# Ladme/groan_rs

Hardware: AMD Instinct MI355X
Metric: frames/sec RMSD-fit, 1e6 atoms triclinic, 1/2/4/8 GPUs; HBM GB/s vs peak (higher is better)
Workload: dtype f32 (fp64 accumulators)

## Files before the change

### groan_rs_amd/csrc/gr_api.hip

```cpp
#include <hip/hip_runtime.h>

#include <cmath>
#include <cstdio>
#include <cstdlib>
#include <cstring>
#include <map>
#include <string>
#include <vector>

#include "../../include/groan_hip.h"
#include "gr_batch.h"
#include "gr_buf.h"
#include "gr_workers.h"
#include "gr_container.h"
#include "gr_kernels.h"
#include "gr_hot.h"
#include "gr_resident.h"
#include "gr_small.h"
#include "gr_xtc.h"
#include "gr_shape.h"
#include "gr_xtc_dev.h"
#include "gr_xtc_enc_dev.h"
#include "gr_trr.h"
#include "gr_cellgrid.h"
#include "gr_textio.h"
#include "gr_pool.h"
#include <set>
#include <thread>
#include <atomic>
#include <system_error>
#include <chrono>

#define GR_MAX_CHUNKS 256

namespace {

struct Group {
    std::vector<grc::Block> blocks;
    uint64_t n = 0;
    bool contiguous = true;
    uint32_t start = 0;
    uint32_t *idx_dev = nullptr;
    uint32_t *mask_dev = nullptr;
    bool walk_rw = false;
    bool masked = false;
    uint32_t span = 0;
};

}

struct GrWhole;

struct gr_ctx {
    int device = 0;
    hipStream_t stream = nullptr;
    hipStream_t copy_stream = nullptr;
    std::vector<hipEvent_t> ev_ready;
    std::vector<uint8_t> upload_pending;
    hipEvent_t ev_done_ring[64] = {};
    uint64_t done_gen = 0;
    std::vector<uint64_t> slot_gen;
    uint32_t *fuse_cnt = nullptr;
    int fuse = 1;
    uint64_t center_fallbacks = 0;
    uint32_t com_onepass_min = 4096;
    uint64_t n = 0, n_pad = 0;
    uint32_t n_slots = 0;
    size_t frame_stride = 0;
    float *frames = nullptr;
    float *aos_up = nullptr;
    float *aos_dl = nullptr;
    float *masses = nullptr;
    std::vector<float> masses_host;
    GrBox *boxes_dev = nullptr;
    GrBox *boxes_host = nullptr;
    std::vector<int> box_status;
    std::vector<uint8_t> box9_set;
    std::vector<float> box9_host;
    std::map<std::string, Group> groups;
    GrWhole *whole = nullptr;
    GrCenPartial *cen_partials = nullptr;
    GrAccPartial *acc_partials = nullptr;
    grbuf::Dev<double> fit_partials;
    int two_pass = 1;
    int masked_sel = 1;
    int rmsd_fast = 1;
    int rmsd_fast_sigmas = 6;
    uint32_t rmsd_fast_min = 16384;
    uint64_t rmsd_fast_frames = 0, rmsd_exact_redos = 0;
    int resident = 1;
    int pd_sym = 1;
    int res_wg_groups = 0;
    int res_streams = 0;
    int res_fill16 = 1;
    uint32_t res_last_streams = 0;
    int res_metro_ns = 1;
    int stream_wgs_cu = 0;
    int translate_rows = 1;
    int center_resident = 1;
    uint64_t cen_res_launches = 0, cen_res_redone = 0;
    int res_fit_last = 0;
    struct Metro { uint64_t shape = 0; double free_ns = 0, T_ns = 0, best_ns = 0, fail_ns = 0; uint32_t off_for = 0, held = 0; } metro;
    uint64_t res_metro_period_ns = 0, res_last_turn_ns = 0, res_late_permille = 0, res_sclk_mhz = 0;
    int wall_khz = 100000;
    uint32_t res_max_wgs = 0;
    int res_test_no_start = 0;
    uint32_t res_test_abort_at = 0xFFFFFFFFu;
    uint32_t res_skip = 0, res_backoff = 0;
    uint32_t *res_progress = nullptr;
    grbuf::Dev<unsigned long long> res_wgrec;
    unsigned long long *res_rec = nullptr;
    uint32_t *res_abort = nullptr;
    uint32_t *res_words_host = nullptr;
    struct ResOut { GrFrameState st[GR_MAX_BATCH]; uint32_t words[16]; alignas(64) uint32_t seq; };
    ResOut *res_out = nullptr, *res_out_dev = nullptr;
    uint32_t res_seq = 0;
    uint32_t res_checkin = 0, res_closed = 0;
    uint32_t res_late_seen[2] = { 0, 0 };
    uint64_t res_lean_segments = 0, res_sync_fallbacks = 0;
    GrShapeSet *shape_set_dev = nullptr;
    grbuf::Dev<unsigned long long> shape_mask_dev; grbuf::Pinned<unsigned long long> shape_mask_host;
    uint32_t res_epoch = 0;
    bool res_in_use = false;
    uint64_t res_launches = 0, res_handshake_misses = 0, res_aborts = 0, res_redone_frames = 0;
    GrFrameState *state_dev = nullptr;
    GrFrameState *state_host = nullptr;
    GrFrameState *small_state = nullptr, *small_state_dev = nullptr;
    uint32_t *small_flag = nullptr, *small_flag_dev = nullptr;
    uint32_t small_seq = 0;
    uint32_t small_max = GR_SMALL_MAX_DEFAULT;
    uint64_t small_calls = 0, small_sync_fallbacks = 0;
    uint32_t *bad_dev = nullptr;
    uint32_t *bad_host = nullptr;
    grbuf::Dev<float> pd_out;
    hipEvent_t ev0 = nullptr, ev1 = nullptr;
    hipEvent_t pev[6 * GR_MAX_BATCH] = {};
    uint32_t sub_batch = 256;
    uint32_t chunks = 0;
    uint32_t fit_wgs = 0;
    int profile = 0;
    double prof_ms[4] = { 0, 0, 0, 0 };
    uint64_t prof_launches[4] = { 0, 0, 0, 0 };
    uint64_t prof_frames[4] = { 0, 0, 0, 0 };
    uint32_t n_cus = 0;
    grbuf::Pinned<unsigned char> xtc_host[2]; grbuf::Dev<unsigned char> xtc_dev[2];
    hipEvent_t xtc_ev[2] = { nullptr, nullptr };
    hipEvent_t xtc_unpacked[2] = { nullptr, nullptr };
    hipStream_t unpack_stream = nullptr;
    uint32_t xtc_bank = 0;
    grbuf::Pinned<float> wr_host;
    grbuf::Dev<unsigned char> xe_dev[6];
    grbuf::Pinned<unsigned char> xe_host[2];
    int xtc_dev_encode = 1;
    uint64_t xtc_dev_frames = 0;
    int strict = 0;
    gr_rmsd_plan *in_flight = nullptr;
    uint32_t in_flight_s0 = 0, in_flight_n = 0;
    uint64_t epoch = 1;
    std::string err;
    uint64_t err_index = 0;
    uint64_t counts[2] = { 0, 0 };
};

struct Pending {
    bool active = false, any_ok = false, consistent = true, fused = false, resident = false, rmsd_fast = false;
    uint32_t res_metro_ns = 0; bool res_metro_auto = false;
    uint32_t s0 = 0, nb = 0, n_prof_groups = 0, res_stream = 0, res_streams = 1;
    int fit = 0;
    std::vector<int> pre;
    std::vector<uint64_t> pre_idx;
    std::vector<std::string> pre_msg;
    GrSel sel = {};
    uint64_t group_n = 0;
    bool has_group = false;
    bool small = false; uint32_t small_seq = 0;
    uint32_t res_seq = 0, res_epoch = 0; bool res_fresh = false;
#ifdef GR_EXP_TIMELINE
    unsigned long long *tl_dev = nullptr;
#endif
};

struct gr_rmsd_plan {
    gr_ctx *target = nullptr;
    Pending pend;
    std::string group;
    uint64_t n_ref = 0;
    float *p_dev = nullptr, *w_dev = nullptr;
    float *p_span_dev = nullptr;
    std::vector<grc::Block> ref_blocks;
    bool span_ok = false;
    std::vector<float> w_host;
    GrPlanDev dev = {};
    int exact = 0;
    bool fit_behind_small = false;
    uint32_t last_fallbacks = 0;
    bool resolved = false;
    uint64_t resolved_epoch = 0;
};

namespace {

thread_local std::string g_create_err;

#define HIPCHK(ctx, call)                                                                      \
    do {                                                                                       \
        hipError_t e_ = (call);                                                                \
        if (e_ != hipSuccess) {                                                                \
            (ctx)->err = std::string(#call) + ": " + hipGetErrorString(e_);                    \
            return GR_E_HIP;                                                                   \
        }                                                                                      \
    } while (0)

int fail(gr_ctx *c, int status, const std::string &msg, uint64_t index = 0) {
    c->err = msg; c->err_index = index; return status;
}

GrSel make_sel(const Group &g) {
    GrSel s;
    s.n = (uint32_t)g.n; s.contiguous = g.contiguous ? 1u : 0u; s.start = g.start; s.g0 = g.start >> 8; s.idx = g.idx_dev;
    s.masked = (g.masked && g.mask_dev) ? (g.walk_rw ? 3u : 1u) : 0u; s.span = g.contiguous ? (uint32_t)g.n : g.span; s.mask = g.mask_dev;
    return s;
}

uint32_t chunks_for(const GrSel &s) {
    const uint64_t units = s.contiguous ? ((uint64_t)s.n + 3) / 4 : (uint64_t)s.n;
    uint64_t c = units / ((uint64_t)GR_WG * 4);
    if (c < 1) c = 1;
    if (c > GR_MAX_CHUNKS) c = GR_MAX_CHUNKS;
    return (uint32_t)c;
}

uint32_t batch_chunks(const gr_ctx *c, const GrSel &s, uint32_t nf) {
    if (c->chunks) return c->chunks;
    const uint64_t units = ((uint64_t)(s.masked ? s.span : s.n) + 3) / 4;
    uint64_t by_work = units / GR_WG;
    if (by_work < 1) by_work = 1;
    uint64_t want = (1536 + nf - 1) / nf;
    if (want < 8) want = 8;
    uint64_t ch = want < by_work ? want : by_work;
    if (ch > GR_MAX_CHUNKS) ch = GR_MAX_CHUNKS;
    if (ch >= 8) ch &= ~(uint64_t)7;
    return (uint32_t)ch;
}

uint32_t fit_grid(const gr_ctx *c, uint32_t nf) {
    (void)nf;
    if (c->fit_wgs) return c->fit_wgs;
    const uint64_t tiles = (c->n + 255) >> 8;
    uint64_t gx = (tiles + GR_WG / 64 - 1) / (GR_WG / 64);
    if (gx >= 8) gx &= ~(uint64_t)7;
    return (uint32_t)(gx < 1 ? 1 : gx);
}

static const void *resident_fn(bool wmass, bool ubox, bool v, bool fl) {
#define GR_RES_FN(W, U, V, F) reinterpret_cast<const void *>(&k_fit_resident<W, U, V, F>)
    static const void *const fn[16] = {
        GR_RES_FN(false, false, false, false), GR_RES_FN(true, false, false, false), GR_RES_FN(false, true, false, false), GR_RES_FN(true, true, false, false),
        GR_RES_FN(false, false, true, false), GR_RES_FN(true, false, true, false), GR_RES_FN(false, true, true, false), GR_RES_FN(true, true, true, false),
        GR_RES_FN(false, false, false, true), GR_RES_FN(true, false, false, true), GR_RES_FN(false, true, false, true), GR_RES_FN(true, true, false, true),
        GR_RES_FN(false, false, true, true), GR_RES_FN(true, false, true, true), GR_RES_FN(false, true, true, true), GR_RES_FN(true, true, true, true) };
#undef GR_RES_FN
    return fn[(wmass ? 1 : 0) | (ubox ? 2 : 0) | (v ? 4 : 0) | (fl ? 8 : 0)];
}
static const void *resident_center_fn(bool ubox, bool fl) {
    static const void *const fn[4] = { reinterpret_cast<const void *>(&k_fit_resident<false, false, false, false, 1>), reinterpret_cast<const void *>(&k_fit_resident<false, true, false, false, 1>),
                                       reinterpret_cast<const void *>(&k_fit_resident<false, false, false, true, 1>), reinterpret_cast<const void *>(&k_fit_resident<false, true, false, true, 1>) };
    return fn[(ubox ? 1 : 0) | (fl ? 2 : 0)];
}
#ifndef GR_STREAM_WGS_CU_DEFAULT
#define GR_STREAM_WGS_CU_DEFAULT 8
// ... 147 lines not shown
    if (!ingest) return busy_check(c);
    if (c->in_flight && slot < c->in_flight_s0 + c->in_flight_n && c->in_flight_s0 < slot + n)
        return fail(c, GR_E_INVALID_ARG, "upload into a slot of the batch in flight: call gr_rmsd_batch_end first (or use the other half of the double buffer)");
    return GR_OK;
}

struct SlotUse {
    gr_ctx *c; uint32_t first, n;
    bool quiet = false;
    SlotUse(gr_ctx *ctx, uint32_t first_slot, uint32_t count = 1) : c(ctx), first(first_slot), n(count) {
        for (uint32_t s = first; s < first + n && s < c->n_slots; ++s)
            if (c->upload_pending[s]) { (void)hipStreamWaitEvent(c->stream, c->ev_ready[s], 0); c->upload_pending[s] = 0; }
    }
    ~SlotUse() {
        if (quiet) return;
        const uint64_t gen = ++c->done_gen;
        (void)hipEventRecord(c->ev_done_ring[gen % 64], c->stream);
        for (uint32_t s = first; s < first + n && s < c->n_slots; ++s) c->slot_gen[s] = gen;
    }
};

static hipError_t sync_ingest(gr_ctx *c) {
    hipError_t e = hipStreamSynchronize(c->copy_stream);
    if (e == hipSuccess && c->unpack_stream) e = hipStreamSynchronize(c->unpack_stream);
    return e;
}
static int slot_box_wait(gr_ctx *c, uint32_t slot) {
    if (c->ev_ready[slot]) HIPCHK(c, hipEventSynchronize(c->ev_ready[slot]));
    else HIPCHK(c, hipEventCreateWithFlags(&c->ev_ready[slot], hipEventDisableTiming));
    return GR_OK;
}
void box_fill(gr_ctx *c, uint32_t slot, const float *box9) {
    GrBox &b = c->boxes_host[slot];
    if (!box9) {
        gr_box_setup(nullptr, &b);
        c->box_status[slot] = GR_E_NO_BOX; c->box9_set[slot] = 0;
    } else {
        const int ok = gr_box_setup(box9, &b);
        memcpy(&c->box9_host[9 * (size_t)slot], box9, 9 * sizeof(float));
        c->box9_set[slot] = 1;
        if (!ok) c->box_status[slot] = GR_E_ZERO_BOX;
        else if (b.ncand > GR_MAX_CAND) c->box_status[slot] = GR_E_UNSUPPORTED_BOX;
        else c->box_status[slot] = GR_OK;
    }
}
int set_box(gr_ctx *c, uint32_t slot, const float *box9, hipStream_t on = nullptr) {
    box_fill(c, slot, box9);
    HIPCHK(c, hipMemcpyAsync(c->boxes_dev + slot, &c->boxes_host[slot], sizeof(GrBox), hipMemcpyHostToDevice, on ? on : c->stream));
    return GR_OK;
}

int set_boxes_same(gr_ctx *c, uint32_t first_slot, uint32_t n, const float *box9, hipStream_t on = nullptr) {
    if (n == 0) return GR_OK;
    float keep[9];
    if (box9) memcpy(keep, box9, sizeof keep);
    box_fill(c, first_slot, box9 ? keep : nullptr);
    for (uint32_t f = 1; f < n; ++f) {
        const uint32_t s = first_slot + f;
        c->boxes_host[s] = c->boxes_host[first_slot];
        c->box_status[s] = c->box_status[first_slot]; c->box9_set[s] = c->box9_set[first_slot];
        if (box9) memcpy(&c->box9_host[9 * (size_t)s], keep, sizeof keep);
    }
    HIPCHK(c, hipMemcpyAsync(c->boxes_dev + first_slot, c->boxes_host + first_slot, (size_t)n * sizeof(GrBox), hipMemcpyHostToDevice, on ? on : c->stream));
    return GR_OK;
}

int ensure_staging(gr_ctx *c, float **buf) {
    if (*buf) return GR_OK;
    HIPCHK(c, hipMalloc(buf, c->frame_stride * sizeof(float)));
    HIPCHK(c, hipMemsetAsync(*buf, 0, c->frame_stride * sizeof(float), c->stream));
    HIPCHK(c, hipStreamSynchronize(c->stream));
    return GR_OK;
}
int untile_slot(gr_ctx *c, uint32_t slot) {
    int st = ensure_staging(c, &c->aos_dl); if (st) return st;
    const uint32_t ng = (uint32_t)(c->n_pad >> 2);
    k_untile<<<dim3((ng + 255) / 256), dim3(256), 0, c->stream>>>(c->frames + (size_t)slot * c->frame_stride, c->aos_dl, ng);
    HIPCHK(c, hipGetLastError());
    return GR_OK;
}

int ensure_event(gr_ctx *c, hipEvent_t *ev, bool timing) {
    if (*ev) return GR_OK;
    HIPCHK(c, timing ? hipEventCreate(ev) : hipEventCreateWithFlags(ev, hipEventDisableTiming));
    return GR_OK;
}
#define EVREC(ctx, ev, timing, stream) do { int s_ = ensure_event((ctx), &(ev), (timing)); if (s_) return s_; HIPCHK((ctx), hipEventRecord((ev), (stream))); } while (0)

int state_reset(gr_ctx *c, uint32_t n) {
    k_state_reset<<<dim3((n + 63) / 64), dim3(64), 0, c->stream>>>(c->state_dev, n);
    HIPCHK(c, hipGetLastError());
    return GR_OK;
}

int fetch_states(gr_ctx *c, uint32_t n) {
    HIPCHK(c, hipMemcpyAsync(c->state_host, c->state_dev, n * sizeof(GrFrameState), hipMemcpyDeviceToHost, c->stream));
    HIPCHK(c, hipStreamSynchronize(c->stream));
    return GR_OK;
}

int frame_status(gr_ctx *c, const GrFrameState &st) {
    if (st.status == GR_OK) return GR_OK;
    if (st.status == GR_E_NO_POSITION) return fail(c, GR_E_NO_POSITION, "atom has no position", st.err_index);
    if (st.status == GR_E_NO_MASS) return fail(c, GR_E_NO_MASS, "atom has no mass", st.err_index);
    return fail(c, st.status, "frame analysis failed");
}

static bool small_ok(const gr_ctx *c, const GrSel &sel) { return c->small_max != 0 && c->small_state != nullptr && sel.n <= c->small_max && !c->profile; }
static int small_wait(gr_ctx *c, uint32_t seq, uint32_t words = 1) {
    volatile uint32_t *w = c->small_flag;
    const auto t0 = std::chrono::steady_clock::now();
    for (uint32_t spins = 0; w[0] != seq || w[words - 1] != seq; ++spins) {
        if ((spins & 1023u) == 1023u && std::chrono::steady_clock::now() - t0 > std::chrono::milliseconds(20)) {
            c->small_sync_fallbacks++;
            HIPCHK(c, hipStreamSynchronize(c->stream));
            if (w[0] != seq || w[words - 1] != seq) return fail(c, GR_E_HIP, "a single-wave kernel ended without publishing its result");
            break;
        }
    }
    std::atomic_thread_fence(std::memory_order_acquire);
    c->small_calls++;
    return GR_OK;
}

static int res_next_epoch(gr_ctx *c, uint32_t *epoch) {
    if (++c->res_epoch == 0u) {
        HIPCHK(c, hipStreamSynchronize(c->stream));
        if (c->res_wgrec.get()) HIPCHK(c, hipMemset(c->res_wgrec.get(), 0, c->res_wgrec.cap() * sizeof(unsigned long long)));
        HIPCHK(c, hipMemset(c->res_rec, 0, (size_t)GR_MAX_BATCH * 16 * sizeof(unsigned long long)));
        HIPCHK(c, hipMemset(c->res_abort + 2, 0, 2 * sizeof(uint32_t)));
        c->res_epoch = 1u;
    }
    *epoch = c->res_epoch;
    return GR_OK;
}
static int res_wgrec_reserve(gr_ctx *c, size_t rec_words, hipStream_t S) {
    bool grew = false;
    HIPCHK(c, c->res_wgrec.reserve(rec_words, grbuf::exact, &grew));
    const hipError_t e = grew ? hipMemsetAsync(c->res_wgrec.get(), 0, rec_words * sizeof(unsigned long long), S) : hipSuccess;
    if (e != hipSuccess) c->res_wgrec.release();
    HIPCHK(c, e);
    return GR_OK;
}
static int res_test_no_start(gr_ctx *c, uint32_t epoch) {
    if (!c->res_test_no_start) return GR_OK;
    const unsigned long long two = 2ull | ((unsigned long long)epoch << 32);
    c->res_test_no_start = 0;
    HIPCHK(c, hipMemcpyAsync(c->res_abort + 2, &two, sizeof two, hipMemcpyHostToDevice, c->stream));
    HIPCHK(c, hipStreamSynchronize(c->stream));
    return GR_OK;
}
template <int MODE>
static int res_close(gr_ctx *c, uint32_t nb, const double *fit_partials, uint32_t nparts, double sum_w, uint32_t epoch, bool fresh, uint32_t *seq) {
    const uint32_t sq = c->res_seq + 1u;
    k_res_close<MODE><<<dim3(nb), dim3(64), 0, c->stream>>>(fit_partials, nparts, sum_w, c->state_dev, c->res_rec, epoch, fresh ? 1u : 0u, c->res_abort, c->res_closed + nb,
                                                        c->res_out_dev->st, c->res_out_dev->words, &c->res_out_dev->seq, sq);
    HIPCHK(c, hipGetLastError());
    c->res_seq = sq; c->res_closed += nb; *seq = sq;
    return GR_OK;
}
static int res_collect(gr_ctx *c, uint32_t seq, uint32_t nb, uint32_t epoch, bool *started) {
    volatile uint32_t *w = &c->res_out->seq;
    const auto t0 = std::chrono::steady_clock::now();
    for (uint32_t spins = 0; *w != seq; ++spins) {
        if ((spins & 1023u) == 1023u && std::chrono::steady_clock::now() - t0 > std::chrono::milliseconds(20)) {
            c->res_sync_fallbacks++;
            HIPCHK(c, hipStreamSynchronize(c->stream));
            if (*w != seq) return fail(c, GR_E_HIP, "the kernel behind the resident pass ended without publishing its results");
            break;
        }
    }
    std::atomic_thread_fence(std::memory_order_acquire);
    memcpy(c->state_host, c->res_out->st, (size_t)nb * sizeof(GrFrameState));
    memcpy(c->res_words_host, c->res_out->words, 12 * sizeof(uint32_t));
    for (int k = 0; k < 2; ++k) { const uint32_t v = c->res_words_host[8 + k]; c->res_words_host[8 + k] = v - c->res_late_seen[k]; c->res_late_seen[k] = v; }
    *started = c->res_words_host[2] == 1u && c->res_words_host[3] == epoch;
    if (!*started || c->res_words_host[0]) HIPCHK(c, hipStreamSynchronize(c->stream));
    return GR_OK;
}

int center_stage(gr_ctx *c, uint32_t first_slot, uint32_t nf, const GrSel &sel, int kind, int weighted,
                 int mass_first, int target, int only_status = 0) {
    if (small_ok(c, sel)) {
        k_center_small_stage<<<dim3(nf), dim3(64), 0, c->stream>>>(c->frames, c->frame_stride, first_slot, c->masses, sel, c->boxes_dev, kind, weighted, mass_first, target, c->state_dev, only_status);
        HIPCHK(c, hipGetLastError());
        return GR_OK;
    }
    uint32_t nch = chunks_for(sel);
    if (nf > 1 && nch >= 8) nch &= ~7u;
    const dim3 grid(nch, nf), wg(GR_WG);
    if (kind == 0) k_center_sums<0><<<grid, wg, 0, c->stream>>>(c->frames, c->frame_stride, first_slot, c->masses, sel, c->boxes_dev, c->state_dev, weighted, c->cen_partials, only_status);
    else if (kind == 1) k_center_sums<1><<<grid, wg, 0, c->stream>>>(c->frames, c->frame_stride, first_slot, c->masses, sel, c->boxes_dev, c->state_dev, weighted, c->cen_partials, only_status);
    else k_center_sums<2><<<grid, wg, 0, c->stream>>>(c->frames, c->frame_stride, first_slot, c->masses, sel, c->boxes_dev, c->state_dev, weighted, c->cen_partials, only_status);
    k_center_finalize<<<dim3(nf), dim3(GR_WG), 0, c->stream>>>(c->cen_partials, nch, c->boxes_dev, first_slot, kind, weighted, mass_first, target, sel.n, c->state_dev, only_status);
    HIPCHK(c, hipGetLastError());
    return GR_OK;
}

int pbc_center_stages(gr_ctx *c, uint32_t first_slot, uint32_t nf, const GrSel &sel, int weighted, int only_status = 0) {
    if (small_ok(c, sel) && only_status == 0) {
        k_center_small_pbc<<<dim3(nf), dim3(64), 0, c->stream>>>(c->frames, c->frame_stride, first_slot, c->masses, sel, c->boxes_dev, weighted, c->state_dev);
        HIPCHK(c, hipGetLastError());
        return GR_OK;
    }
    int st = center_stage(c, first_slot, nf, sel, 1, 0, 0, 0, only_status);
    if (st != GR_OK) return st;
    return center_stage(c, first_slot, nf, sel, 2, weighted, 0, 1, only_status);
}

static bool center_onepass_ok(const gr_ctx *c, const GrSel &sel) {
    return c->com_onepass_min != 0 && (sel.contiguous || sel.masked) && sel.n >= c->com_onepass_min && c->two_pass;
}
static int pbc_center_onepass(gr_ctx *c, uint32_t s0, uint32_t nb, const GrSel &sel, int weighted) {
    GrPlanDev plan; memset(&plan, 0, sizeof plan);
    plan.w_is_mass = weighted ? 1u : 0u;
    plan.n = sel.n; plan.sw = 1.0;
    const uint32_t nch = batch_chunks(c, sel, nb);
    if (sel.masked) {
        k_sums_pk<true, false, true><<<dim3(nch, nb), dim3(GR_WG), 0, c->stream>>>(c->frames, c->frame_stride, s0, c->masses, sel, c->boxes_dev, plan, c->acc_partials,
                                                                                   c->fuse ? c->fuse_cnt : nullptr, c->fuse ? c->state_dev : nullptr);
        if (!c->fuse) k_rmsd_finalize_lite<true><<<dim3(nb), dim3(64), 0, c->stream>>>(c->acc_partials, nch, c->frames, c->frame_stride, s0, sel, c->boxes_dev, plan, c->state_dev);
    } else if (c->fuse) {
        k_sums_pk<true><<<dim3(nch, nb), dim3(GR_WG), 0, c->stream>>>(c->frames, c->frame_stride, s0, c->masses, sel, c->boxes_dev, plan, c->acc_partials, c->fuse_cnt, c->state_dev);
    } else {
        k_sums_pk<true><<<dim3(nch, nb), dim3(GR_WG), 0, c->stream>>>(c->frames, c->frame_stride, s0, c->masses, sel, c->boxes_dev, plan, c->acc_partials, nullptr, nullptr);
        k_rmsd_finalize_lite<true><<<dim3(nb), dim3(64), 0, c->stream>>>(c->acc_partials, nch, c->frames, c->frame_stride, s0, sel, c->boxes_dev, plan, c->state_dev);
    }
    HIPCHK(c, hipGetLastError());
    return GR_OK;
}
static int center_redo_fallbacks(gr_ctx *c, uint32_t s0, uint32_t nb, const GrSel &sel, int weighted, std::vector<GrFrameState> &res) {
    uint32_t n_fb = 0, n_amb = 0;
    for (uint32_t f = 0; f < nb; ++f) { n_fb += c->state_host[f].status == GR_ST_FALLBACK; n_amb += c->state_host[f].status == GR_ST_AMBIG; }
    if (n_fb || n_amb) {
        c->center_fallbacks += n_fb + n_amb;
        int st = GR_OK;
        if (n_amb) { st = center_stage(c, s0, nb, sel, 1, 0, 0, 0, GR_ST_AMBIG); if (st) return st; }
        if (n_fb) { st = pbc_center_stages(c, s0, nb, sel, weighted, GR_ST_FALLBACK); if (st) return st; }
        st = fetch_states(c, nb); if (st) return st;
    }
    res.assign(c->state_host, c->state_host + nb);
    return GR_OK;
}

}

static int gr_abi_guard() { return GR_E_HIP; }

extern "C" {

const char *gr_version(void) { return "groan_hip 0.1.0 (gfx950)"; }

const char *gr_status_string(int s) try {
    switch (s) {
    case GR_OK: return "ok";
    case GR_E_NO_BOX: return "simulation box does not exist";
    case GR_E_NOT_ORTHOGONAL: return "simulation box is not orthogonal";
    case GR_E_ZERO_BOX: return "box length is zero or negative";
    case GR_E_EMPTY_GROUP: return "group is empty";
    case GR_E_INCONSISTENT_GROUP: return "group has a different number of atoms in reference and target";
    case GR_E_NO_POSITION: return "atom has undefined position";
    case GR_E_NO_MASS: return "atom has undefined mass";
    case GR_E_GROUP_NOT_FOUND: return "group does not exist";
    case GR_E_OUT_OF_RANGE: return "atom index out of range";
    case GR_E_INVALID_ARG: return "invalid argument";
    case GR_E_GROUP_EXISTS: return "group already existed and was overwritten";
    case GR_E_HIP: return "HIP runtime error";
    case GR_E_NO_DEVICE: return "no usable HIP device";
    case GR_E_UNSUPPORTED_BOX: return "box too skewed for the minimum-image table";
    case GR_E_IO: return "file could not be opened or read";
    case GR_E_FORMAT: return "not a valid xtc file";
    case GR_E_INVALID_NAME: return "invalid group name";
    case GR_E_EMPTY_CHAIN: return "no acceptor and no donor atoms detected for chain";
    case GR_E_NONEXISTENT_CHAIN: return "chain does not exist";
    case GR_E_DUPLICATE_PAIR: return "pair of chains requested multiple times";
    case GR_E_UNUSED_CHAIN: return "not all chains are used";
    case GR_E_INVALID_BOND: return "invalid bond";
    case GR_E_INVALID_SPAN: return "invalid span of the grid map";
    case GR_E_INVALID_TILE: return "invalid grid tile";
    default: return "unknown status";
    }
} catch (...) { return nullptr; }

int gr_device_count(int *count) try {
    int n = 0;
    if (hipGetDeviceCount(&n) != hipSuccess) { if (count) *count = 0; return GR_E_NO_DEVICE; }
    if (count) *count = n;
    return n > 0 ? GR_OK : GR_E_NO_DEVICE;
} catch (...) { return gr_abi_guard(); }

gr_ctx *gr_ctx_create(int device, uint64_t n_atoms, uint32_t n_slots, int *status) try {
    int dummy; if (!status) status = &dummy;
    int ndev = 0;
    if (hipGetDeviceCount(&ndev) != hipSuccess || ndev <= 0 || device < 0 || device >= ndev) { *status = GR_E_NO_DEVICE; return nullptr; }
    if (n_atoms == 0 || n_atoms > 0xFFFFFFF0ull || n_slots == 0) { *status = GR_E_INVALID_ARG; return nullptr; }
    if (hipSetDevice(device) != hipSuccess) { *status = GR_E_NO_DEVICE; return nullptr; }
    gr_ctx *c = new gr_ctx();
    c->device = device; c->n = n_atoms; c->n_pad = (n_atoms + 255) & ~255ull; c->n_slots = n_slots;
    c->frame_stride = (size_t)c->n_pad * 3;
    bool ok = true;
    ok = ok && hipStreamCreateWithFlags(&c->stream, hipStreamNonBlocking) == hipSuccess;
    ok = ok && hipStreamCreateWithFlags(&c->copy_stream, hipStreamNonBlocking) == hipSuccess;
    for (int k = 0; k < 64; ++k) ok = ok && hipEventCreateWithFlags(&c->ev_done_ring[k], hipEventDisableTiming) == hipSuccess;
    c->ev_ready.assign(n_slots, nullptr); c->upload_pending.assign(n_slots, 0); c->slot_gen.assign(n_slots, 0);
    ok = ok && hipMalloc(&c->fuse_cnt, 2 * GR_MAX_BATCH * sizeof(uint32_t)) == hipSuccess;
    ok = ok && hipMemset(c->fuse_cnt, 0, 2 * GR_MAX_BATCH * sizeof(uint32_t)) == hipSuccess;
    { hipDeviceProp_t prop; if (hipGetDeviceProperties(&prop, device) == hipSuccess) c->n_cus = (uint32_t)prop.multiProcessorCount; }
    ok = ok && hipMalloc(&c->frames, (size_t)n_slots * c->frame_stride * sizeof(float)) == hipSuccess;
    ok = ok && hipMalloc(&c->masses, c->n_pad * sizeof(float)) == hipSuccess;
    ok = ok && hipMalloc(&c->boxes_dev, n_slots * sizeof(GrBox)) == hipSuccess;
    ok = ok && hipHostMalloc(&c->boxes_host, n_slots * sizeof(GrBox), hipHostMallocDefault) == hipSuccess;
// ... 2623 lines not shown
```

### groan_rs_amd/csrc/gr_resident.h

```cpp
#pragma once
#include <type_traits>
#include "gr_hot.h"

struct GrResShape {
    static constexpr int LANES = 512, WAVES = LANES / 64;
#ifndef GR_RES_K
#define GR_RES_K 6
#endif
    static constexpr int K = GR_RES_K;
    static constexpr int R = 8;
    static constexpr int PARK_F4 = K * 3 * LANES;
    static constexpr int WSUM_F = R * WAVES * 32;
#ifdef GR_EXP_TIMELINE
    static constexpr int TL_BYTES = 128 * 4 * 8;
#else
    static constexpr int TL_BYTES = 0;
#endif
    static constexpr int LDS_BYTES = PARK_F4 * 16 + WSUM_F * 4 + R * WAVES * 8 + 3 * R * 4 + 2 * WAVES * 4 + TL_BYTES;
    static constexpr int REC_PER_WAVE = 256 / WAVES, LANES_PER_REC = 64 / REC_PER_WAVE, WORDS_PER_LANE = 32 / LANES_PER_REC;
};
#ifndef GR_RES_SLEEP
#define GR_RES_SLEEP 2
#endif
#ifndef GR_RES_BAL
// ... 792 lines not shown
            }
        } else if (status == 0) {
            GrResRot T;
            T.r00 = rec.r00; T.r10 = rec.r10; T.r20 = rec.r20; T.r01 = rec.r01; T.r11 = rec.r11; T.r21 = rec.r21;
            T.r02 = rec.r02; T.r12 = rec.r12; T.r22 = rec.r22;
            if (V) {
                const float t0x = rec.t0x, t0y = rec.t0y, t0z = rec.t0z;
                T.sx = T.sy = T.sz = 0.f;
                fit_group_v(GA, ra, T, t0x, t0y, t0z, oa, rs);
                if (GB.valid) fit_group_v(GB, rb, T, t0x, t0y, t0z, ob, rs);
            } else {
                T.sx = rec.sx; T.sy = rec.sy; T.sz = rec.sz;
                const GrBox *boxp = boxes + first_slot + kf(j);
                gr_res_fit_group<WMASS>(GA, ra.r0, ra.r1, ra.r2, T, B, boxp, cx, cy, cz, oa.r0, oa.r1, oa.r2, rs);
                if (GB.valid) gr_res_fit_group<WMASS>(GB, rb.r0, rb.r1, rb.r2, T, B, boxp, cx, cy, cz, ob.r0, ob.r1, ob.r2, rs);
            }
        }
        {
#ifdef GR_EXP_NOSTORE
            const __amdgpu_buffer_rsrc_t out = gr_buf_rsrc(frames + (size_t)(first_slot + kf(j)) * frame_stride, 0u);
#else
            const __amdgpu_buffer_rsrc_t out = gr_buf_rsrc(frames + (size_t)(first_slot + kf(j)) * frame_stride, status == 0 ? slot_bytes : 0u);
#endif
            gr_buf_store_stream(out, offA, oa.r0); gr_buf_store_stream(out, offA + 1024u, oa.r1); gr_buf_store_stream(out, offA + 2048u, oa.r2);
            gr_buf_store_stream(out, offB, ob.r0); gr_buf_store_stream(out, offB + 1024u, ob.r1); gr_buf_store_stream(out, offB + 2048u, ob.r2);
        }
        n_fitted = j + 1u;
        if (MODE == 1) return;
        const float wtot = gr_wave_allsum_f32(rs);
        if (lane == 0) fit_partials[((size_t)kf(j) * ctl.wgs_frame + wg) * WAVES + wave] = (double)wtot;
    };

    Landing L0, L1;
    L0.a.r0 = L0.a.r1 = L0.a.r2 = L0.b.r0 = L0.b.r1 = L0.b.r2 = zero4; L0.gx = L0.gy = L0.gz = 0.f;
    L1 = L0;
    Rows Q0, Q1, Q2, Q3, Q4, Q5;
    Q0.r0 = Q0.r1 = Q0.r2 = zero4; Q1 = Q0; Q2 = Q0; Q3 = Q0; Q4 = Q0; Q5 = Q0;
    unsigned long long rv = 0ull;
    gate(0);
    if (n_turns) request(0, L0);
    const uint32_t n_iter = n_turns + K;
    const GrBoxU B0 = gr_box_uniform(boxes + first_slot);
    auto lds_put = [&](uint32_t slot, const Rows &rw) { park[(slot * 3 + 0) * LANES + tid] = rw.r0; park[(slot * 3 + 1) * LANES + tid] = rw.r1; park[(slot * 3 + 2) * LANES + tid] = rw.r2; };
    auto lds_get = [&](uint32_t slot) { Rows rw; rw.r0 = park[(slot * 3 + 0) * LANES + tid]; rw.r1 = park[(slot * 3 + 1) * LANES + tid]; rw.r2 = park[(slot * 3 + 2) * LANES + tid]; return rw; };
    auto step_sums_first = [&](uint32_t i, Landing &cur, Landing &nxt) {
        rv = request_rec(i >= K && i < n_iter ? i - K : 0u);
#ifdef GR_EXP_NOLOAD
        if (i < 2) request(i + 1, nxt);
#else
        GR_STEP_STAMP(6);
        gate(i + 1);
        GR_STEP_STAMP(0);
        request(i + 1, nxt);
#endif
        balance(i);
        const GrBoxU Bf = UBOX ? B0 : gr_box_uniform(boxes + first_slot + kf(i >= K ? i - K : 0u));
        const GrBoxU Bs = UBOX ? B0 : gr_box_uniform(boxes + first_slot + kf(i < n_turns ? i : 0u));
        Rows va = cur.a, vb = cur.b;
        const uint32_t ps = i % K;
        GR_STEP_STAMP(1);
        if (i < n_turns) { if constexpr (MODE == 1) sums_cen(i, cur, Bs); else sums(i, cur, Bs, va, vb); }
#if GR_RES_LATE_COMBINE
        if (i == n_turns && n_turns > 0u && claim(n_turns - 1u)) { if constexpr (MODE == 1) combine_cen(n_turns - 1u); else combine_rmsd(n_turns - 1u); }
#endif
        GR_STEP_STAMP(3);
        if (i >= K) {
            Rows qb;
            if (ps == 0u) { qb = Q0; asm volatile("; set 0 out"); } else if (ps == 1u) { qb = Q1; asm volatile("; set 1 out"); } else if (ps == 2u) { qb = Q2; asm volatile("; set 2 out"); }
            else if (ps == 3u) { qb = Q3; asm volatile("; set 3 out"); } else if (ps == 4u) { qb = Q4; asm volatile("; set 4 out"); } else { qb = Q5; asm volatile("; set 5 out"); }
            fit(i - K, rv, lds_get(ps), qb, Bf);
            if (bail) return;
        }
        GR_STEP_STAMP(5);
        if (i < n_turns) {
            lds_put(ps, va);
            if (ps == 0u) { Q0 = vb; asm volatile("; set 0 in"); } else if (ps == 1u) { Q1 = vb; asm volatile("; set 1 in"); } else if (ps == 2u) { Q2 = vb; asm volatile("; set 2 in"); }
            else if (ps == 3u) { Q3 = vb; asm volatile("; set 3 in"); } else if (ps == 4u) { Q4 = vb; asm volatile("; set 4 in"); } else { Q5 = vb; asm volatile("; set 5 in"); }
        }
    };
    auto step_fit_first = [&](uint32_t i, Landing &cur, Landing &nxt) {
#ifdef GR_EXP_NOLOAD
        if (i < 2) request(i + 1, nxt);
#elif !defined(GR_EXP_LATE_REQUEST)
        gate(i + 1);
        request(i + 1, nxt);
#endif
        balance(i);
        const GrBoxU Bf = UBOX ? B0 : gr_box_uniform(boxes + first_slot + kf(i >= K ? i - K : 0u));
        const GrBoxU Bs = UBOX ? B0 : gr_box_uniform(boxes + first_slot + kf(i < n_turns ? i : 0u));
        Rows va = cur.a, vb = cur.b;
        const uint32_t ps = i % K;
        if (i >= K) {
            Rows qb;
            if (ps == 0u) { qb = Q0; asm volatile("; set 0 out"); } else if (ps == 1u) { qb = Q1; asm volatile("; set 1 out"); } else if (ps == 2u) { qb = Q2; asm volatile("; set 2 out"); }
            else if (ps == 3u) { qb = Q3; asm volatile("; set 3 out"); } else if (ps == 4u) { qb = Q4; asm volatile("; set 4 out"); } else { qb = Q5; asm volatile("; set 5 out"); }
            fit(i - K, rv, lds_get(ps), qb, Bf);
            if (bail) return;
        }
        rv = request_rec(i + 1 >= K && i + 1 < n_iter ? i + 1 - K : 0u);
#ifdef GR_EXP_LATE_REQUEST
        request(i + 1, nxt);
#endif
        if (i < n_turns) {
            if (MODE == 1) sums_cen(i, cur, Bs);
            else if (V) sums(i, cur, Bs, va, vb);
            lds_put(ps, va);
            if (ps == 0u) { Q0 = vb; asm volatile("; set 0 in"); } else if (ps == 1u) { Q1 = vb; asm volatile("; set 1 in"); } else if (ps == 2u) { Q2 = vb; asm volatile("; set 2 in"); }
            else if (ps == 3u) { Q3 = vb; asm volatile("; set 3 in"); } else if (ps == 4u) { Q4 = vb; asm volatile("; set 4 in"); } else { Q5 = vb; asm volatile("; set 5 in"); }
            if (!V && MODE != 1) sums(i, cur, Bs, va, vb);
        }
#if GR_RES_LATE_COMBINE
        if (i == n_turns && n_turns > 0u && claim(n_turns - 1u)) { if constexpr (MODE == 1) combine_cen(n_turns - 1u); else combine_rmsd(n_turns - 1u); }
#endif
    };
    auto step = [&](uint32_t i, Landing &cur, Landing &nxt) { if constexpr (FL) step_sums_first(i, cur, nxt); else step_fit_first(i, cur, nxt); };
    for (uint32_t i = 0; i < n_iter && !bail; i += 2) {
        step(i, L0, L1);
        if (!bail && i + 1 < n_iter) step(i + 1, L1, L0);
    }
    if (lane == 0) {
        ctl.progress[wg_all * WAVES + wave] = n_fitted;
        (void)__hip_atomic_fetch_max(reinterpret_cast<unsigned long long *>(ctl.abort + 6), (unsigned long long)wall_clock64(), __ATOMIC_RELAXED, __HIP_MEMORY_SCOPE_AGENT);
        if (n_late) (void)__hip_atomic_fetch_add(ctl.abort + 8, n_late, __ATOMIC_RELAXED, __HIP_MEMORY_SCOPE_AGENT);
        if (n_waited) (void)__hip_atomic_fetch_add(ctl.abort + 9, n_waited, __ATOMIC_RELAXED, __HIP_MEMORY_SCOPE_AGENT);
#ifdef GR_EXP_STEPTIME
        if (ctl.dbg) {
            unsigned long long *o = ctl.dbg + (size_t)(wg_all * WAVES + wave) * 4u;
            unsigned long long tot = 0; for (int k = 0; k < 7; ++k) tot += st_acc[k];
            o[0] = st_acc[4]; o[1] = st_acc[7] | (st_combines << 32);
            o[2] = (__builtin_amdgcn_s_getreg((20 << 0) | (0 << 6) | (3 << 11)) & 7u) | (simd_of[wave] << 8);
            o[3] = tot;
        }
        if ((wg_all == 0u || wg_all == ctl.n_stream / 2u) && (wave == 0u || wave == 5u)) {
            unsigned long long *o = reinterpret_cast<unsigned long long *>(ctl.abort + 16) + ((wg_all ? 2u : 0u) + (wave ? 1u : 0u)) * 8u;
            for (int k = 0; k < 8; ++k) o[k] = st_acc[k];
        }
#endif
        if (clk_wave) {
            const unsigned long long dc = (unsigned long long)clock64() - clk_c0, dw = (unsigned long long)wall_clock64() - clk_w0;
            gr_st_agent(ctl.abort + 10, (uint32_t)(dc >> 8)); gr_st_agent(ctl.abort + 11, (uint32_t)(dw >> 8));
        }
    }
#ifdef GR_EXP_TIMELINE
    if (tl_wg && wave == 0 && !bail) {
        for (uint32_t t = (n_turns > 128u ? n_turns - 128u : 0u) + lane; t < n_turns; t += 64u) {
            const size_t f = kf(t);
            ctl.tl[f * 8 + 0] = tls[(t & 127u) * 4u + 0u];
            ctl.tl[f * 8 + 6] = tls[(t & 127u) * 4u + 1u] | (tls[(t & 127u) * 4u + 2u] << 48);
        }
    }
#endif
}

template <int MODE>
__global__ __launch_bounds__(64) void k_res_close(const double *__restrict__ fit_partials, uint32_t nparts, double sum_w, GrFrameState *state,
                                                  const unsigned long long *__restrict__ rec, uint32_t epoch, uint32_t fresh_states, uint32_t *ctl_words,
                                                  uint32_t done_target, GrFrameState *out_states, uint32_t *out_words, uint32_t *out_seq, uint32_t seq) {
    constexpr uint32_t NW = sizeof(GrFrameState) / 4u, W_RMSD = offsetof(GrFrameState, rmsd) / 4u, W_STATUS = offsetof(GrFrameState, status) / 4u;
    static_assert(sizeof(GrFrameState) % 4u == 0 && NW <= 64u, "a frame state is exported by one wave, a word per lane");
    const uint32_t frame = blockIdx.x, lane = threadIdx.x;
    uint32_t *sw = reinterpret_cast<uint32_t *>(state + frame);
    uint32_t w = 0u;
    if (fresh_states && (uint32_t)(gr_ld_agent(rec + (size_t)frame * 16u) >> 32) != epoch) {
        GrFrameState z = {};
        z.err_index = GR_NOIDX; z.status = GR_ST_ABORTED;
        if (lane < NW) { w = reinterpret_cast<const uint32_t *>(&z)[lane]; sw[lane] = w; }
    } else if (lane < NW) w = sw[lane];
    const int status = __shfl((int)w, (int)W_STATUS, 64);
    if (MODE == 0 && status == 0) {
        double s0 = 0.0, s1 = 0.0, s2 = 0.0, s3 = 0.0;
        const double *p = fit_partials + (size_t)frame * nparts;
        uint32_t k = lane;
        for (; k + 192 < nparts; k += 256) { s0 += p[k]; s1 += p[k + 64]; s2 += p[k + 128]; s3 += p[k + 192]; }
        for (; k < nparts; k += 64) s0 += p[k];
        const double s = gr_wave_sum((s0 + s1) + (s2 + s3));
        float r = 0.0f;
        if (lane == 0) { r = (float)sqrt(fmax(s, 0.0) / sum_w); state[frame].rmsd = r; }
        r = __shfl(r, 0, 64);
        if (lane == W_RMSD) w = __float_as_uint(r);
    }
    if (lane < NW) reinterpret_cast<uint32_t *>(out_states + frame)[lane] = w;
    __threadfence_system();
    uint32_t n = 0u;
    if (lane == 0) n = __hip_atomic_fetch_add(ctl_words + 12, 1u, __ATOMIC_ACQ_REL, __HIP_MEMORY_SCOPE_AGENT) + 1u;
    n = (uint32_t)__builtin_amdgcn_readfirstlane((int)n);
    if (n != done_target) return;
    if (lane < 12u) out_words[lane] = gr_ld_agent(ctl_words + lane);
    __threadfence_system();
    if (lane == 0) __hip_atomic_store(out_seq, seq, __ATOMIC_RELEASE, __HIP_MEMORY_SCOPE_SYSTEM);
}
```

Baseline: 140,700.

## Split resident close into per-frame reduce and single-block export kernel

The per-frame close kernel no longer publishes its state to host-visible memory or counts finished blocks with an atomic to pick the last one. A separate single-workgroup export kernel now copies all frame states and control words and then releases the sequence word. The close kernel also issues all fit-partial loads up front into registers, before the status check, so load latency overlaps the state read. This costs an extra kernel launch and more register use per wave, in exchange for dropping the per-block system fences and the atomic counter.

```diff
diff --git a/groan_rs_amd/csrc/gr_api.hip b/groan_rs_amd/csrc/gr_api.hip
--- a/groan_rs_amd/csrc/gr_api.hip
+++ b/groan_rs_amd/csrc/gr_api.hip
@@ -115,7 +115,7 @@
     struct ResOut { GrFrameState st[GR_MAX_BATCH]; uint32_t words[16]; alignas(64) uint32_t seq; };
     ResOut *res_out = nullptr, *res_out_dev = nullptr;
     uint32_t res_seq = 0;
-    uint32_t res_checkin = 0, res_closed = 0;
+    uint32_t res_checkin = 0;
     uint32_t res_late_seen[2] = { 0, 0 };
     uint64_t res_lean_segments = 0, res_sync_fallbacks = 0;
     GrShapeSet *shape_set_dev = nullptr;
@@ -569,11 +569,12 @@
 }
 template <int MODE>
 static int res_close(gr_ctx *c, uint32_t nb, const double *fit_partials, uint32_t nparts, double sum_w, uint32_t epoch, bool fresh, uint32_t *seq) {
+    static_assert(GR_MAX_BATCH <= GR_RES_EXPORT_FRAMES, "k_res_export copies the states of one segment");
     const uint32_t sq = c->res_seq + 1u;
-    k_res_close<MODE><<<dim3(nb), dim3(64), 0, c->stream>>>(fit_partials, nparts, sum_w, c->state_dev, c->res_rec, epoch, fresh ? 1u : 0u, c->res_abort, c->res_closed + nb,
-                                                        c->res_out_dev->st, c->res_out_dev->words, &c->res_out_dev->seq, sq);
+    k_res_close<MODE><<<dim3(nb), dim3(64), 0, c->stream>>>(fit_partials, nparts, sum_w, c->state_dev, c->res_rec, epoch, fresh ? 1u : 0u);
+    k_res_export<<<dim3(1), dim3(GR_RES_EXPORT_LANES), 0, c->stream>>>(c->state_dev, nb, c->res_abort, c->res_out_dev->st, c->res_out_dev->words, &c->res_out_dev->seq, sq);
     HIPCHK(c, hipGetLastError());
-    c->res_seq = sq; c->res_closed += nb; *seq = sq;
+    c->res_seq = sq; *seq = sq;
     return GR_OK;
 }
 static int res_collect(gr_ctx *c, uint32_t seq, uint32_t nb, uint32_t epoch, bool *started) {
diff --git a/groan_rs_amd/csrc/gr_resident.h b/groan_rs_amd/csrc/gr_resident.h
--- a/groan_rs_amd/csrc/gr_resident.h
+++ b/groan_rs_amd/csrc/gr_resident.h
@@ -968,40 +968,73 @@
 #endif
 }
 
+#define GR_RES_CLOSE_LOADS 32
 template <int MODE>
 __global__ __launch_bounds__(64) void k_res_close(const double *__restrict__ fit_partials, uint32_t nparts, double sum_w, GrFrameState *state,
-                                                  const unsigned long long *__restrict__ rec, uint32_t epoch, uint32_t fresh_states, uint32_t *ctl_words,
-                                                  uint32_t done_target, GrFrameState *out_states, uint32_t *out_words, uint32_t *out_seq, uint32_t seq) {
-    constexpr uint32_t NW = sizeof(GrFrameState) / 4u, W_RMSD = offsetof(GrFrameState, rmsd) / 4u, W_STATUS = offsetof(GrFrameState, status) / 4u;
-    static_assert(sizeof(GrFrameState) % 4u == 0 && NW <= 64u, "a frame state is exported by one wave, a word per lane");
+                                                  const unsigned long long *__restrict__ rec, uint32_t epoch, uint32_t fresh_states) {
+    constexpr uint32_t NW = sizeof(GrFrameState) / 4u, W_STATUS = offsetof(GrFrameState, status) / 4u, W_ERRIDX = offsetof(GrFrameState, err_index) / 4u;
+    constexpr int NL = GR_RES_CLOSE_LOADS;
+    static_assert(sizeof(GrFrameState) % 4u == 0 && NW <= 64u && NL % 4 == 0, "a frame state is one wave's, a word per lane; the fit sums go four chains at a time");
     const uint32_t frame = blockIdx.x, lane = threadIdx.x;
     uint32_t *sw = reinterpret_cast<uint32_t *>(state + frame);
-    uint32_t w = 0u;
-    if (fresh_states && (uint32_t)(gr_ld_agent(rec + (size_t)frame * 16u) >> 32) != epoch) {
-        GrFrameState z = {};
-        z.err_index = GR_NOIDX; z.status = GR_ST_ABORTED;
-        if (lane < NW) { w = reinterpret_cast<const uint32_t *>(&z)[lane]; sw[lane] = w; }
-    } else if (lane < NW) w = sw[lane];
+    const double *p = fit_partials + (size_t)frame * nparts;
+    const bool flat = MODE == 0 && nparts != 0u && nparts <= (uint32_t)NL * 64u;
+    const uint32_t tag = (uint32_t)(gr_ld_agent(rec + (size_t)frame * 16u) >> 32);
+    uint32_t w = lane < NW ? sw[lane] : 0u;
+    double v[NL];
+    if (flat) {
+#pragma unroll
+        for (int j = 0; j < NL; ++j) { const uint32_t k = lane + 64u * (uint32_t)j; v[j] = p[k < nparts ? k : nparts - 1u]; }
+        __builtin_amdgcn_sched_barrier(0);
+    }
+    if (fresh_states && tag != epoch) {
+        w = lane == W_STATUS ? (uint32_t)GR_ST_ABORTED : lane == W_ERRIDX ? (uint32_t)GR_NOIDX : 0u;
+        if (lane < NW) sw[lane] = w;
+    }
     const int status = __shfl((int)w, (int)W_STATUS, 64);
     if (MODE == 0 && status == 0) {
         double s0 = 0.0, s1 = 0.0, s2 = 0.0, s3 = 0.0;
-        const double *p = fit_partials + (size_t)frame * nparts;
-        uint32_t k = lane;
-        for (; k + 192 < nparts; k += 256) { s0 += p[k]; s1 += p[k + 64]; s2 += p[k + 128]; s3 += p[k + 192]; }
-        for (; k < nparts; k += 64) s0 += p[k];
+        if (flat) {
+#pragma unroll
+            for (int g = 0; g < NL / 4; ++g) {
+                const uint32_t k = lane + 256u * (uint32_t)g;
+                if (k + 192u < nparts) { s0 += v[4 * g]; s1 += v[4 * g + 1]; s2 += v[4 * g + 2]; s3 += v[4 * g + 3]; }
+                else {
+                    if (k < nparts) s0 += v[4 * g];
+                    if (k + 64u < nparts) s0 += v[4 * g + 1];
+                    if (k + 128u < nparts) s0 += v[4 * g + 2];
+                }
+            }
+        } else {
+            uint32_t k = lane;
+            for (; k + 192 < nparts; k += 256) { s0 += p[k]; s1 += p[k + 64]; s2 += p[k + 128]; s3 += p[k + 192]; }
+            for (; k < nparts; k += 64) s0 += p[k];
+        }
         const double s = gr_wave_sum((s0 + s1) + (s2 + s3));
-        float r = 0.0f;
-        if (lane == 0) { r = (float)sqrt(fmax(s, 0.0) / sum_w); state[frame].rmsd = r; }
-        r = __shfl(r, 0, 64);
-        if (lane == W_RMSD) w = __float_as_uint(r);
-    }
-    if (lane < NW) reinterpret_cast<uint32_t *>(out_states + frame)[lane] = w;
+        if (lane == 0) state[frame].rmsd = (float)sqrt(fmax(s, 0.0) / sum_w);
+    }
+}
+
+#define GR_RES_EXPORT_LANES 1024
+#define GR_RES_EXPORT_FRAMES 1024
+__global__ __launch_bounds__(GR_RES_EXPORT_LANES) void k_res_export(const GrFrameState *__restrict__ state, uint32_t nb, const uint32_t *ctl_words,
+                                                                     GrFrameState *out_states, uint32_t *out_words, uint32_t *out_seq, uint32_t seq) {
+    constexpr uint32_t W64 = sizeof(GrFrameState) / 8u, PER = (GR_RES_EXPORT_FRAMES * W64 + GR_RES_EXPORT_LANES - 1u) / GR_RES_EXPORT_LANES;
+    static_assert(sizeof(GrFrameState) % 8u == 0, "the states are copied as 64-bit words");
+    const uint32_t nw = (nb < GR_RES_EXPORT_FRAMES ? nb : GR_RES_EXPORT_FRAMES) * W64;
+    if (nw == 0u) return;
+    const unsigned long long *src = reinterpret_cast<const unsigned long long *>(state);
+    unsigned long long *dst = reinterpret_cast<unsigned long long *>(out_states);
+    unsigned long long v[PER];
+#pragma unroll
+    for (uint32_t j = 0; j < PER; ++j) { const uint32_t i = threadIdx.x + j * GR_RES_EXPORT_LANES; v[j] = src[i < nw ? i : nw - 1u]; }
+    const uint32_t cw = threadIdx.x < 12u ? gr_ld_agent(ctl_words + threadIdx.x) : 0u;
+#pragma unroll
+    for (uint32_t j = 0; j < PER; ++j) { const uint32_t i = threadIdx.x + j * GR_RES_EXPORT_LANES; if (i < nw) __hip_atomic_store(dst + i, v[j], __ATOMIC_RELAXED, __HIP_MEMORY_SCOPE_SYSTEM); }
+    if (threadIdx.x < 12u) __hip_atomic_store(out_words + threadIdx.x, cw, __ATOMIC_RELAXED, __HIP_MEMORY_SCOPE_SYSTEM);
+    asm volatile("s_waitcnt vmcnt(0)" ::: "memory");
+    __syncthreads();
+    if (threadIdx.x >= 64u) return;
     __threadfence_system();
-    uint32_t n = 0u;
-    if (lane == 0) n = __hip_atomic_fetch_add(ctl_words + 12, 1u, __ATOMIC_ACQ_REL, __HIP_MEMORY_SCOPE_AGENT) + 1u;
-    n = (uint32_t)__builtin_amdgcn_readfirstlane((int)n);
-    if (n != done_target) return;
-    if (lane < 12u) out_words[lane] = gr_ld_agent(ctl_words + lane);
-    __threadfence_system();
-    if (lane == 0) __hip_atomic_store(out_seq, seq, __ATOMIC_RELEASE, __HIP_MEMORY_SCOPE_SYSTEM);
+    if (threadIdx.x == 0) __hip_atomic_store(out_seq, seq, __ATOMIC_RELEASE, __HIP_MEMORY_SCOPE_SYSTEM);
 }
```

New measurement: 142,400, median of 6. About the same (+1.2%).
